# san-soucie/gdrf

Measured on AMD Instinct MI355X. Metric: ELBO steps/sec (+ achieved HBM GB/s on K_nm) at N=1e6,M=512,K=10,V=50, higher is better.
Workload: dtype f32

## Files before the change

gdrf_amd/csrc/api.hip:

```cpp
#include "../../include/gdrf_hip.h"
#include "common.h"
#include "gemm_nt.h"
#include "gemm_tn.h"
#include "gemm_split.h"
#include "gemm_tn_topics.h"
#include "gemm_tn_topics1.h"
#include "kernels_mm.h"
#include "kernels_n.h"
#include "predict.h"
#include "rows_mfma.h"
#include "rows_vstream.h"
#include "hyper_tn.h"
#include "optim.h"

#include <algorithm>
#include <cmath>
#include <cstdio>
#include <cstdlib>
#include <cstring>
#include <string>
#include <type_traits>
#include <vector>

using namespace gdrf;
// ... 950 lines not shown
    if (mask & SL_TRANSFORMS) {
      ScopedTimer tm(c, 2, s);
      dim3 g3((Mp + 255) / 256, Mp, K);
      hipLaunchKernelGGL(build_s_kernel<T>, g3, dim3(256), 0, s, Sunc, M, Mp, P(c->S), P(c->ST));
      hipLaunchKernelGGL(build_phi_kernel<T>, dim3(K), dim3(64), 0, s, phi_unc, K, V, P(c->phi));
      if (c->unwhitened) {
        if ((rc = unwhiten_forward(c, U, s))) return rc;
        U = (const T*)c->Uw;
      }
      hipLaunchKernelGGL(build_upad_kernel<T>, dim3((Mp + 255) / 256, GDRF_TILE), dim3(256), 0, s, U, K, M, Mp, P(c->Upad));
      if (!c->Tst && (rc = mm_nt<T>(c, P(c->S), mm, P(c->S), mm, P(c->Bm), mm, T(1), K, s))) return rc;
      if constexpr (std::is_same<T, float>::value) {
        if (c->split) {
          const SplitLay SL{K};
          HIPCHK(hipMemsetAsync(c->smx, 0, (size_t)SL.nmax() * sizeof(unsigned), s));
          if (c->split == 2) {
            hipLaunchKernelGGL(absmax_batched_kernel, dim3(64, K), dim3(256), 0, s, (const float*)c->Bm, mm, mm, c->smx + SL.mx_b(0));
            hipLaunchKernelGGL(absmax_batched_kernel, dim3(64, K), dim3(256), 0, s, (const float*)c->ST, mm, mm, c->smx + SL.mx_st(0));
          }
          split_scales(c, SPLIT_SC_W | SPLIT_SC_BST, s);
        }
      }
    }
    const int64_t rtiles = (n + GDRF_TILE - 1) / GDRF_TILE;
    if (mask & SL_FORWARD) {
    {
      if ((rc = knm_solve(c, X, n, s))) return rc;
      if ((rc = join_fact(c, s))) return rc;
      ScopedTimer tm(c, 3, s);
      FwdWProb<TS, T> p{{}, {}, (const TS*)Q(c->Knm), n, Mp, (const TS*)Q(c->Linv), P(c->W), P(c->qpart), ldk};
      if (c->split && sizeof(TS) == 8 && sizeof(T) == 4) {
        p.Wh = c->Wh; p.wh_stride = (int64_t)c->ncap * Mp; p.wh_mode = c->split; p.wh_scale = c->ssc + SplitLay{K}.w();
      }
      hipLaunchKernelGGL((gemm_nt_kernel<TS, FwdWProb<TS, T>>), dim3(nt_xcd_row_grid(rtiles, nct<TS>(c))), dim3(256), CS::LDS_BYTES, s, p);
    }
    HIPCHK(hipEventRecord(c->ev_fork, s));
    HIPCHK(hipStreamWaitEvent(c->side, c->ev_fork, 0));
    {
      ScopedTimer tm(c, 4, c->side);
      const size_t ulds = (size_t)K * Mp * sizeof(T);
      if (K <= LOC_KMAX && Mp % (16 * Vec16<T>::N) == 0 && ulds <= 150 * 1024) {
        if (ulds > 48 * 1024) HIPCHK(hipFuncSetAttribute((const void*)loc_rows_kernel<T>, hipFuncAttributeMaxDynamicSharedMemorySize, (int)ulds));
        const int64_t blocks = std::min<int64_t>((n + 31) / 32, 256 * 8);
        hipLaunchKernelGGL(loc_rows_kernel<T>, dim3((unsigned)blocks), dim3(256), ulds, c->side, (const T*)P(c->W), n, Mp, K, (const T*)P(c->Upad), P(c->loc), ldk);
      } else {
        bool wide = false;
        if constexpr (sizeof(T) == 8) {
          if (K > C::CW) {
            LocProb<T, true> p{{}, {}, {}, P(c->W), n, Mp, K, P(c->Upad), P(c->loc), ldk};
            hipLaunchKernelGGL((gemm_nt_kernel<T, LocProb<T, true>>), dim3((unsigned)rtiles), dim3(256), C::LDS_BYTES, c->side, p);
            wide = true;
          }
        }
        if (!wide) {
          LocProb<T> p{{}, {}, {}, P(c->W), n, Mp, K, P(c->Upad), P(c->loc), ldk};
          hipLaunchKernelGGL((gemm_nt_kernel<T, LocProb<T>>), dim3((unsigned)rtiles), dim3(256), C::LDS_BYTES, c->side, p);
        }
      }
    }
    HIPCHK(hipEventRecord(c->ev_loc, c->side));
    if constexpr (std::is_same<T, float>::value && sizeof(TS) == 8) {
      if (hyper_tn_on(c) && !(mask & SL_NO_DK)) {
        const int vpr = Mp / 8, rpp = 256 / vpr;
        const int64_t blocks = std::min<int64_t>((n + rpp - 1) / rpp, 256 * 16);
        if (!c->dKh) {
          void* pw = nullptr;
          hipError_t e = hipMalloc(&pw, (size_t)2 * c->ncap * Mp * 2);
// ... 133 lines not shown
        dim3 gr1((Mp + 255) / 256, Mp, 1);
        hipLaunchKernelGGL(reduce_slabs_kernel<T>, gr1, dim3(256), 0, ss, (const T*)slab_gt, ns, 1, Mp, 0, redT + roff(c, 3)); }
    }
    HIPCHK(hipEventRecord(c->ev_join, c->side));
    bool hyper_done = false;
    if constexpr (std::is_same<T, float>::value && sizeof(TS) == 8) {
      if (hyper_tn_on(c)) {
        hipStream_t ss = c->side;
        ScopedTimer tm(c, 8, ss);
        const int BR = TNCfg<T>::BR;
        const int ns = std::min(tn_nsplit_gt(c, n, BR), c->nsplit_cap);
        const int64_t rps = round_up((n + ns - 1) / ns, BR);
        float* slab_hd = (float*)c->slab + (int64_t)c->nsplit_cap * (K + 1) * mm;
        const SplitLay SL{K};
        if ((rc = tn_split<SplitF16>(c, (const float*)c->Wbar, nullptr, 0, n, rps, 0, slab_hd, 1, ns, c->nt * c->nt, SL.wbar(), 0, ss, c->dKh, SL.dk()))) return rc;
        hipLaunchKernelGGL(slab_linvt_dot_kernel<TS>, dim3((unsigned)M), dim3(256), 0, ss, (const float*)slab_hd, ns, Mp, M, (const TS*)Q(c->LinvT), c->hpart);
        hipLaunchKernelGGL(reduce_dparts_kernel, dim3(1), dim3(1024), 0, ss, c->hpart, (int64_t)M, 1, redd + 5);
        hipLaunchKernelGGL(wbar_w_dot_kernel<T>, dim3(2048), dim3(256), 0, ss, (const T*)P(c->Wbar), (const T*)P(c->W), n, Mp, c->hpart + Mp);
        hipLaunchKernelGGL(reduce_dparts_kernel, dim3(1), dim3(1024), 0, ss, c->hpart + Mp, (int64_t)2048, 1, redd + 4);
        HIPCHK(hipMemsetAsync(redd + 6, 0, sizeof(double), ss));
        LAUNCHCHK("hyper_tn");
        HIPCHK(hipEventRecord(c->ev_join, c->side));
        hyper_done = true;
      }
    }
    if (!hyper_done) {
      ScopedTimer tm(c, 8, s);
      const int64_t nb = nt_xcd_row_grid(rtiles, nct<TS>(c));
      if (3 * nb > c->dpart_len) return fail(-1, "gdrf_step_local", "n_local exceeds the context capacity");
      if (c->per) {
        if (c->learn_z) {
          BwdKnmProb<TS, T, true, true, true> p{{}, {}, P(c->Wbar), n, M, Mp, c->D, c->kind, (const TS*)Q(c->LinvT), (const TS*)Q(c->Knm), X,
                                                (const TS*)Q(c->Zs), c->hyp, c->dpart, c->zpart, c->apart, Xr, (const TS*)Q(c->Zph)};
          hipLaunchKernelGGL((gemm_nt_kernel<TS, BwdKnmProb<TS, T, true, true, true>>), dim3((unsigned)nb), dim3(256), CS::LDS_BYTES, s, p);
          hipLaunchKernelGGL(reduce_parts_kernel<double>, dim3((unsigned)((M * c->D + 255) / 256)), dim3(256), 0, s, (const double*)c->zpart, rtiles,
                             (int64_t)M * c->D, redd + 8);
        } else {
          BwdKnmProb<TS, T, false, true, true> p{{}, {}, P(c->Wbar), n, M, Mp, c->D, c->kind, (const TS*)Q(c->LinvT), (const TS*)Q(c->Knm), X,
                                                 (const TS*)Q(c->Zs), c->hyp, c->dpart, nullptr, c->apart, Xr, (const TS*)Q(c->Zph)};
          if (sizeof(TS) == 8)
            hipLaunchKernelGGL((gemm_nt_kernel_v160<TS, BwdKnmProb<TS, T, false, true, true>>), dim3((unsigned)nb), dim3(256), CS::LDS_BYTES, s, p);
          else hipLaunchKernelGGL((gemm_nt_kernel<TS, BwdKnmProb<TS, T, false, true, true>>), dim3((unsigned)nb), dim3(256), CS::LDS_BYTES, s, p);
        }
        hipLaunchKernelGGL(reduce_dparts_kernel, dim3(1), dim3(1024), 0, s, c->apart, nb, c->D + c->npair, redd + 8 + (int64_t)M * c->D);
      } else if (c->ard) {
        if (c->learn_z) {
          BwdKnmProb<TS, T, true, true> p{{}, {}, P(c->Wbar), n, M, Mp, c->D, c->kind, (const TS*)Q(c->LinvT), (const TS*)Q(c->Knm), X, (const TS*)Q(c->Zs),
                                          c->hyp, c->dpart, c->zpart, c->apart};
          hipLaunchKernelGGL((gemm_nt_kernel<TS, BwdKnmProb<TS, T, true, true>>), dim3((unsigned)nb), dim3(256), CS::LDS_BYTES, s, p);
          hipLaunchKernelGGL(reduce_parts_kernel<double>, dim3((unsigned)((M * c->D + 255) / 256)), dim3(256), 0, s, (const double*)c->zpart, rtiles,
                             (int64_t)M * c->D, redd + 8);
        } else {
          BwdKnmProb<TS, T, false, true> p{{}, {}, P(c->Wbar), n, M, Mp, c->D, c->kind, (const TS*)Q(c->LinvT), (const TS*)Q(c->Knm), X, (const TS*)Q(c->Zs),
                                           c->hyp, c->dpart, nullptr, c->apart};
          if (sizeof(TS) == 8) hipLaunchKernelGGL((gemm_nt_kernel_v160<TS, BwdKnmProb<TS, T, false, true>>), dim3((unsigned)nb), dim3(256), CS::LDS_BYTES, s, p);
          else hipLaunchKernelGGL((gemm_nt_kernel<TS, BwdKnmProb<TS, T, false, true>>), dim3((unsigned)nb), dim3(256), CS::LDS_BYTES, s, p);
        }
        hipLaunchKernelGGL(reduce_dparts_kernel, dim3(1), dim3(1024), 0, s, c->apart, nb, c->D, redd + 8 + (int64_t)M * c->D);
      } else if (c->learn_z) {
        BwdKnmProb<TS, T, true> p{{}, {}, P(c->Wbar), n, M, Mp, c->D, c->kind, (const TS*)Q(c->LinvT), (const TS*)Q(c->Knm), X, (const TS*)Q(c->Zs),
                                  c->hyp, c->dpart, c->zpart};
        hipLaunchKernelGGL((gemm_nt_kernel<TS, BwdKnmProb<TS, T, true>>), dim3((unsigned)nb), dim3(256), CS::LDS_BYTES, s, p);
        hipLaunchKernelGGL(reduce_parts_kernel<double>, dim3((unsigned)((M * c->D + 255) / 256)), dim3(256), 0, s, (const double*)c->zpart, rtiles,
                           (int64_t)M * c->D, redd + 8);
      } else {
        BwdKnmProb<TS, T> p{{}, {}, P(c->Wbar), n, M, Mp, c->D, c->kind, (const TS*)Q(c->LinvT), (const TS*)Q(c->Knm), X, (const TS*)Q(c->Zs), c->hyp,
                            c->dpart, nullptr};
        if (sizeof(TS) == 8) hipLaunchKernelGGL((gemm_nt_kernel_v160<TS, BwdKnmProb<TS, T>>), dim3((unsigned)nb), dim3(256), CS::LDS_BYTES, s, p);
        else hipLaunchKernelGGL((gemm_nt_kernel<TS, BwdKnmProb<TS, T>>), dim3((unsigned)nb), dim3(256), CS::LDS_BYTES, s, p);
      }
      hipLaunchKernelGGL(reduce_dparts_kernel, dim3(1), dim3(1024), 0, s, c->dpart, nb, 3, redd + 4);
    }
    LAUNCHCHK("backward");
    {
      const int BR = TNCfg<T>::BR;
      const int ns = std::min(tn_nsplit(c, n, BR, c->split ? 2 : 3), c->nsplit_cap);
      const int64_t rps = round_up((n + ns - 1) / ns, BR);
      TNArgs<T> a{P(c->W), Mp, P(c->W), Mp, P(c->vbar), ldk, n, rps, Mp, 1, P(c->slab), K, ns};
      int red_ns = ns, red_qd = GDRF_TILE / 2;
      { ScopedTimer tm(c, 9, s);
        if (c->split == 2) {
          if constexpr (std::is_same<T, float>::value) {
            const SplitLay SL{K};
            const int nst = std::min(tn_topics_nsplit(c, n), c->nsplit_cap);
            const int64_t rpst = round_up((n + nst - 1) / nst, 32);
            const int ntl = tnt_ntiles(Mp), kgroups = (K + TNT_KT - 1) / TNT_KT;
            TNTopicsArgs ta{(const _Float16*)c->Wh, (int64_t)c->ncap * Mp, Mp, (const float*)c->W, Mp, (const float*)c->vbar, ldk, n, rpst, Mp,
                            (float*)c->slab, K, nst, ntl, (const float*)c->ssc, SL.w(), SL.v(0)};
            if (10 * K >= 6 * kgroups * TNT_KT) {
              int ns1 = c->nsplit_cap < 64 ? c->nsplit_cap : 64;
              while (ns1 > 8 && (n + ns1 - 1) / ns1 < 8 * TN1_CH) ns1 -= 8;
              if (ns1 >= 8) ns1 &= ~7;
              const int64_t rps1 = round_up((n + ns1 - 1) / ns1, TN1_CH);
              const int64_t lds64 = round_up(c->ncap, 64);
              hipLaunchKernelGGL(tn1_scale_rows_kernel, dim3(256, K), dim3(256), 0, s, (const float*)c->vbar, ldk, n, (float*)c->vbs, lds64,
                                 (const float*)c->ssc, SL.v(0));
              TNTopicsArgs t1{(const _Float16*)c->Wh, (int64_t)c->ncap * Mp, Mp, (const float*)c->W, Mp, (const float*)c->vbs, lds64, n, rps1, Mp,
                              (float*)c->slab, K, ns1, ntl, (const float*)c->ssc, SL.w(), SL.v(0)};
              const int nth = tn2_ntiles_half(Mp);
              TNTopicsArgs t0 = t1, t4 = t1;
              t0.ntiles = ntl - nth; t4.ntiles = nth;
              HIPCHK(hipFuncSetAttribute((const void*)tn_topics_w2_kernel<0>, hipFuncAttributeMaxDynamicSharedMemorySize, tn2_lds_bytes()));
// ... 587 lines not shown
```

gdrf_amd/csrc/common.h:

```cpp
#pragma once
#include <hip/hip_runtime.h>
#include <stdint.h>

#define GDRF_WAVE 64
#define GDRF_TILE 128
#define GDRF_KBYTES 128
#define GDRF_FWDW_WGS 2
#define GDRF_FWDW_DEPTH 2
#define GDRF_MPAD 32
#define GDRF_DMAX 4

namespace gdrf {

template <typename T> struct Vec16;
template <> struct Vec16<float>  { using type = float  __attribute__((ext_vector_type(4))); static constexpr int N = 4; };
template <> struct Vec16<double> { using type = double __attribute__((ext_vector_type(2))); static constexpr int N = 2; };

template <typename T> struct Mfma;
template <> struct Mfma<float> {
  using acc_t = float __attribute__((ext_vector_type(4)));
  static __device__ __forceinline__ acc_t mma(float a, float b, acc_t c) {
    return __builtin_amdgcn_mfma_f32_16x16x4f32(a, b, c, 0, 0, 0);
  }
  static __device__ __forceinline__ int crow(int lane, int r) { return ((lane >> 4) << 2) + r; }
};
template <> struct Mfma<double> {
  using acc_t = double __attribute__((ext_vector_type(4)));
  static __device__ __forceinline__ acc_t mma(double a, double b, acc_t c) {
    return __builtin_amdgcn_mfma_f64_16x16x4f64(a, b, c, 0, 0, 0);
  }
  static __device__ __forceinline__ int crow(int lane, int r) { return (lane >> 4) + (r << 2); }
};

__device__ __forceinline__ void gdrf_raw_barrier() {
  asm volatile("" ::: "memory");
  __builtin_amdgcn_s_barrier();
  asm volatile("" ::: "memory");
}

template <typename T> __device__ __forceinline__ T wave_sum(T v) {
#pragma unroll
  for (int o = 32; o > 0; o >>= 1) v += __shfl_xor(v, o, 64);
  return v;
}
template <typename T> __device__ __forceinline__ T group16_sum(T v) {
// ... 81 lines not shown
```

gdrf_amd/csrc/gemm_nt.h:

```cpp
#pragma once
#include "common.h"

namespace gdrf {

template <typename T> struct NTCfg {
  static constexpr int BK = GDRF_KBYTES / (int)sizeof(T);
  static constexpr int VE = 16 / (int)sizeof(T);
  static constexpr int LDK = BK + VE;
  static constexpr int KG = BK / 4;
  static constexpr int VPR = BK / VE;
  static constexpr int VPT = GDRF_TILE * VPR / 256;
  static constexpr int CW = sizeof(T) == 4 ? 128 : 64;
  static constexpr int NB = CW / 32;
  static constexpr int VPTB = CW * VPR / 256;
  static constexpr int LDS_BYTES = (GDRF_TILE + CW) * LDK * (int)sizeof(T);
};

template <typename T> __device__ __forceinline__ int nt_stage_row(int i) { return (int)(threadIdx.x / NTCfg<T>::VPR) + (256 / NTCfg<T>::VPR) * i; }
template <typename T> __device__ __forceinline__ int nt_stage_k() { return (int)(threadIdx.x % NTCfg<T>::VPR) * NTCfg<T>::VE; }

template <class P, class = void> struct NTTri { static constexpr int value = 0; };
template <class P> struct NTTri<P, decltype((void)P::TRI)> { static constexpr int value = P::TRI; };

template <class P, class = void> struct NTMinWgs { static constexpr int value = 2; };
template <class P> struct NTMinWgs<P, decltype((void)P::MIN_WGS)> { static constexpr int value = P::MIN_WGS; };

template <typename T, class P> __device__ __forceinline__ void gemm_nt_body(P& p);

template <typename T, class P>
__global__ __launch_bounds__(256, NTMinWgs<P>::value) void gemm_nt_kernel(P p) { gemm_nt_body<T, P>(p); }

template <typename T, class P>
__global__ __launch_bounds__(256, 3) __attribute__((amdgpu_num_vgpr(80))) void gemm_nt_kernel_v160(P p) { gemm_nt_body<T, P>(p); }

template <typename T, class P>
__device__ __forceinline__ void gemm_nt_body(P& p) {
  using C = NTCfg<T>;
  using V = typename Vec16<T>::type;
  using MM = Mfma<T>;
  using acc_t = typename MM::acc_t;
  extern __shared__ __attribute__((aligned(16))) char smem[];
  T* As = reinterpret_cast<T*>(smem);
  T* Bs = As + GDRF_TILE * C::LDK;
  char* extra = smem + C::LDS_BYTES;

  const int tid = threadIdx.x, lane = tid & 63, wave = tid >> 6;
  const int wr = wave >> 1, wc = wave & 1, lr = lane & 15, lg = lane >> 4;
  const int wc_u = __builtin_amdgcn_readfirstlane(wc);
  const int nct = p.col_tiles();
  const bool loopc = p.loop_cols();
  int64_t rtile; int ct_first;
  p.map_block(blockIdx.x, nct, loopc, rtile, ct_first);
  const int ct_last = loopc ? nct : ct_first + 1;
  const int64_t m0 = rtile * GDRF_TILE;
  const int bz = p.batch_index(blockIdx.x, blockIdx.y);
  const int R = p.a_reuse();

  typename P::ACtx actx;
  p.prepA(actx, m0, bz, extra);
  typename P::ECtx ectx;
  p.prepE(ectx, m0, bz);
  const T* scaleS = reinterpret_cast<const T*>(extra);

  const int srow_k = nt_stage_k<T>();
  for (int ct = ct_first; ct < ct_last; ++ct) {
    const int n0 = ct * C::CW;
    acc_t acc[4][C::NB];
#pragma unroll
    for (int a = 0; a < 4; ++a)
#pragma unroll
      for (int b = 0; b < C::NB; ++b) acc[a][b] = acc_t{0, 0, 0, 0};
    int kb, ke;
    p.krange(m0, n0, bz, kb, ke);
    const int nchunks = (ke > kb) ? ((ke - kb) / C::BK) * R : 0;
    const int nk = (ke > kb) ? (ke - kb) / C::BK : 0;
    auto chunk_pos = [&](int c, int& kA, int& rep) {
      if (P::A_PER_REP) { rep = c / nk; kA = kb + (c - rep * nk) * C::BK; }
      else { const int q = c / R; rep = c - q * R; kA = kb + q * C::BK; }
    };
    typename P::AVec ra0[C::VPT], ra1[C::VPT];
    V rb0[C::VPTB], rb1[C::VPTB];
    auto gload = [&](typename P::AVec (&ra)[C::VPT], V (&rb)[C::VPTB], int c) {
      int kA, rep;
      chunk_pos(c, kA, rep);
      if (rep == 0 || P::A_PER_REP) {
#pragma unroll
        for (int i = 0; i < C::VPT; ++i) ra[i] = p.loadA(actx, i, kA + srow_k, rep, bz);
      }
#pragma unroll
      for (int i = 0; i < C::VPTB; ++i) rb[i] = p.loadB(n0, i, kA + srow_k, rep, bz);
    };
    auto compute = [&](int rep, int kA = 0) {
      T sc[4];
      bool need[C::NB];
#pragma unroll
      for (int b = 0; b < C::NB; ++b) {
        const int c0 = n0 + wc_u * (C::CW / 2) + b * 16;
        need[b] = NTTri<P>::value == 1 ? (kA <= c0 + 15) : (NTTri<P>::value == 2 ? (kA + C::BK - 1 >= c0) : true);
      }
      if (P::SCALE_A) {
#pragma unroll
        for (int t4 = 0; t4 < 4; ++t4) sc[t4] = rep >= 0 ? scaleS[rep * GDRF_TILE + wr * 64 + t4 * 16 + lr] : T(1);
      }
      const T* pa = &As[(wr * 64 + lr) * C::LDK + lg * C::KG];
      const T* pb = &Bs[(wc * (C::CW / 2) + lr) * C::LDK + lg * C::KG];
#pragma unroll
      for (int v = 0; v < C::KG / C::VE; ++v) {
        V fa[4], fb[C::NB];
#pragma unroll
        for (int t4 = 0; t4 < 4; ++t4) {
          fa[t4] = *reinterpret_cast<const V*>(pa + t4 * 16 * C::LDK + v * C::VE);
          if (P::SCALE_A) {
#pragma unroll
            for (int e = 0; e < C::VE; ++e) fa[t4][e] *= sc[t4];
          }
        }
#pragma unroll
        for (int t4 = 0; t4 < C::NB; ++t4) fb[t4] = *reinterpret_cast<const V*>(pb + t4 * 16 * C::LDK + v * C::VE);
#pragma unroll
        for (int e = 0; e < C::VE; ++e)
#pragma unroll
          for (int a = 0; a < 4; ++a)
#pragma unroll
            for (int b = 0; b < C::NB; ++b) {
              if (NTTri<P>::value == 0 || need[b]) acc[a][b] = MM::mma(fa[a][e], fb[b][e], acc[a][b]);
            }
      }
    };
    auto body = [&](typename P::AVec (&ra)[C::VPT], V (&rb)[C::VPTB], int c) {
      int kA, rep;
      chunk_pos(c, kA, rep);
      __syncthreads();
      if (rep == 0 || P::A_PER_REP) {
#pragma unroll
        for (int i = 0; i < C::VPT; ++i) *reinterpret_cast<V*>(&As[nt_stage_row<T>(i) * C::LDK + srow_k]) = p.a_to_lds(ra[i], actx, i, kA + srow_k);
      }
#pragma unroll
      for (int i = 0; i < C::VPTB; ++i) *reinterpret_cast<V*>(&Bs[nt_stage_row<T>(i) * C::LDK + srow_k]) = rb[i];
      __syncthreads();
      if (c + P::DEPTH < nchunks) gload(ra, rb, c + P::DEPTH);
      compute(rep, kA);
    };
    if (P::DEPTH == 1) {
      if (nchunks > 0) gload(ra0, rb0, 0);
      for (int c = 0; c < nchunks; ++c) body(ra0, rb0, c);
    } else {
      if (nchunks > 0) gload(ra0, rb0, 0);
      if (nchunks > 1) gload(ra1, rb1, 1);
      for (int c = 0; c < nchunks; c += 2) {
        body(ra0, rb0, c);
        if (c + 1 < nchunks) body(ra1, rb1, c + 1);
      }
    }
    for (int x = 0; x < p.extra_chunks(); ++x) {
      __syncthreads();
      p.fill_extra(As, Bs, x, m0, n0);
      __syncthreads();
      compute(-1);
    }
    p.tile_done(acc, m0, n0, bz, ectx, wr, wc, lane);
  }
  p.finish(m0, bz, ectx, smem, wr, wc, lane);
}

template <typename T> __device__ __forceinline__ int nt_acc_row(int wr, int a, int lane, int r) {
  return wr * 64 + a * 16 + Mfma<T>::crow(lane, r);
}
template <typename T> __device__ __forceinline__ int nt_acc_col(int wc, int b, int lane) {
  return wc * (NTCfg<T>::CW / 2) + b * 16 + (lane & 15);
}

template <typename T> struct NTPlainA {
  using AVec = typename Vec16<T>::type;
  template <class... X> __device__ __forceinline__ AVec a_to_lds(const AVec& v, X&&...) const { return v; }
};
struct NTNoExtra {
  __device__ __forceinline__ int extra_chunks() const { return 0; }
  template <typename T> __device__ __forceinline__ void fill_extra(T*, T*, int, int64_t, int) const {}
};

struct NTDefaultMap {
  __device__ __forceinline__ int batch_index(unsigned, unsigned by) const { return (int)by; }
  __device__ __forceinline__ void map_block(unsigned bid, int nct, bool loopc, int64_t& rtile, int& ct) const {
    if (loopc) { rtile = bid; ct = 0; } else { rtile = bid / nct; ct = (int)(bid % nct); }
  }
};
struct NTXcdMap {
  __device__ __forceinline__ int batch_index(unsigned, unsigned by) const { return (int)by; }
  __device__ __forceinline__ void map_block(unsigned bid, int nct, bool loopc, int64_t& rtile, int& ct) const {
    if (loopc) { rtile = bid; ct = 0; return; }
    if (nct > 8 || (8 % nct) != 0 || (gridDim.x % 8u) != 0) { rtile = bid / nct; ct = (int)(bid % nct); return; }
    const unsigned xcd = bid & 7u, idx = bid >> 3, per = 8u / (unsigned)nct;
    ct = (int)(xcd % (unsigned)nct);
    rtile = (int64_t)idx * per + xcd / (unsigned)nct;
  }
};

inline unsigned nt_xcd_row_grid(int64_t rtiles, int nct) { return (unsigned)(8 * nct * ((rtiles + 7) / 8)); }
struct NTXcdRowMap {
  __device__ __forceinline__ int batch_index(unsigned, unsigned by) const { return (int)by; }
  __device__ __forceinline__ void map_block(unsigned bid, int nct, bool loopc, int64_t& rtile, int& ct) const {
    if (loopc) { rtile = bid; ct = 0; return; }
    const unsigned xcd = bid & 7u, idx = bid >> 3;
    rtile = (int64_t)(idx / (unsigned)nct) * 8 + xcd;
    ct = (int)(idx % (unsigned)nct);
    if ((nct & 3) == 0 && ((idx >> 2) & 1u)) ct = (ct & ~3) + 3 - (ct & 3);
  }
};

struct NTXcdRowBatchMap {
  int nbatch;
  __device__ __forceinline__ int batch_index(unsigned bid, unsigned) const { return (int)((bid >> 3) % (unsigned)nbatch); }
// ... 51 lines not shown
```

gdrf_amd/csrc/gemm_split.h:

```cpp
#pragma once
#include "common.h"
#include "gemm_nt.h"
#include "kernels_mm.h"

namespace gdrf {

typedef __bf16 bf16x8 __attribute__((ext_vector_type(8)));
typedef __bf16 bf16x4 __attribute__((ext_vector_type(4)));
typedef _Float16 f16x8 __attribute__((ext_vector_type(8)));
typedef _Float16 f16x4 __attribute__((ext_vector_type(4)));
typedef float f32x4 __attribute__((ext_vector_type(4)));
typedef uint32_t u32x4 __attribute__((ext_vector_type(4)));

struct SplitBf16 {
  using E = __bf16; using V8 = bf16x8; using V4 = bf16x4;
  static constexpr int NP = 3, NPROD = 6, ID = 1;
  static __device__ __forceinline__ constexpr int pa(int t) { constexpr int v[6] = {0, 1, 2, 0, 1, 0}; return v[t]; }
  static __device__ __forceinline__ constexpr int pb(int t) { constexpr int v[6] = {2, 1, 0, 1, 0, 0}; return v[t]; }
  static __device__ __forceinline__ f32x4 mma(V8 a, V8 b, f32x4 c) { return __builtin_amdgcn_mfma_f32_16x16x32_bf16(a, b, c, 0, 0, 0); }
  static __device__ __forceinline__ void split(float x, E (&p)[NP]) {
    p[0] = (__bf16)x;
    const float r1 = x - (float)p[0];
    p[1] = (__bf16)r1;
    p[2] = (__bf16)(r1 - (float)p[1]);
// ... 45 lines not shown
  if ((what & SPLIT_SC_WBAR) && t == 0) put(L.wbar(), f16 ? split_pow2_scale(__uint_as_float(mx[L.mx_wbar()]), 15) : 1.0f);
  for (int k = t; k < K; k += blockDim.x) {
    if (what & SPLIT_SC_BST) {
      put(L.b(k), f16 ? split_pow2_scale(__uint_as_float(mx[L.mx_b(k)]), 15) : 1.0f);
      put(L.st(k), f16 ? split_pow2_scale(__uint_as_float(mx[L.mx_st(k)]), 15) : 1.0f);
    }
    if (what & SPLIT_SC_V) put(L.v(k), f16 ? split_pow2_scale(__uint_as_float(mx[L.mx_v(k)]) * sqrtf((float)h->var), 13) : 1.0f);
  }
}
__global__ __launch_bounds__(256) void absmax_batched_kernel(const float* __restrict__ x, int64_t n, int64_t ld, unsigned* __restrict__ mx) {
  const int b = blockIdx.y;
  float m = 0;
  const f32x4* p = reinterpret_cast<const f32x4*>(x + (int64_t)b * ld);
  for (int64_t i = (int64_t)blockIdx.x * blockDim.x + threadIdx.x; i < (n >> 2); i += (int64_t)gridDim.x * blockDim.x) {
    const f32x4 v = p[i];
    m = fmaxf(fmaxf(m, fmaxf(fabsf(v[0]), fabsf(v[1]))), fmaxf(fabsf(v[2]), fabsf(v[3])));
  }
  if (blockIdx.x == 0 && threadIdx.x < (n & 3)) m = fmaxf(m, fabsf(x[(int64_t)b * ld + (n & ~(int64_t)3) + threadIdx.x]));
#pragma unroll
  for (int o = 32; o > 0; o >>= 1) m = fmaxf(m, __shfl_xor(m, o, 64));
  if ((threadIdx.x & 63) == 0 && m > 0) atomicMax(mx + b, __float_as_uint(m));
}

template <class SP> struct SplitCfg {
  static constexpr int BK = 32;
  static constexpr int LDH = BK;
  static constexpr int PIECE = GDRF_TILE * LDH;
  static constexpr int IMG = SP::NP * PIECE;
  static constexpr int LDS_BYTES = 2 * IMG * 2;
};
__device__ __forceinline__ int split_swz(int row) { return (row & 8) ? 3 : 0; }
__device__ __forceinline__ int split_off(int row, int k) { return row * 32 + (((k >> 3) ^ split_swz(row)) << 3) + (k & 7); }

__device__ __forceinline__ void glds16_asm(const void* gsrc, unsigned lds_dst) {
  asm volatile("s_mov_b32 m0, %1\n\ts_nop 0\n\tglobal_load_lds_dwordx4 %0, off" : : "v"(gsrc), "s"(lds_dst) : "memory");
}
__device__ __forceinline__ void glds16_asm_s(const void* sbase, unsigned voff, unsigned lds_dst) {
  asm volatile("s_mov_b32 m0, %2\n\ts_nop 0\n\tglobal_load_lds_dwordx4 %0, %1" : : "v"(voff), "s"(sbase), "s"(lds_dst) : "memory");
}
__device__ __forceinline__ unsigned lds_addr(const void* p) {
  return (unsigned)(uintptr_t)(__attribute__((address_space(3))) const void*)p;
}


template <class SP>
__global__ void split_kernel(const float* __restrict__ in, int64_t n, typename SP::E* __restrict__ out, int64_t stride, const float* __restrict__ scale) {
  const int64_t i = ((int64_t)blockIdx.x * blockDim.x + threadIdx.x) * 4;
  if (i >= n) return;
  const float s = scale[0];
  const f32x4 x = *reinterpret_cast<const f32x4*>(in + i);
  typename SP::V4 pv[SP::NP];
#pragma unroll
  for (int e = 0; e < 4; ++e) {
    typename SP::E p[SP::NP];
    SP::split(x[e] * s, p);
#pragma unroll
    for (int q = 0; q < SP::NP; ++q) pv[q][e] = p[q];
  }
#pragma unroll
  for (int q = 0; q < SP::NP; ++q) *reinterpret_cast<typename SP::V4*>(out + q * stride + i) = pv[q];
}

template <class SP>
__global__ void split_blocked_kernel(const float* __restrict__ in, int64_t n, int R, int C, typename SP::E* __restrict__ out, int64_t stride,
                                     const float* __restrict__ scale) {
  const int64_t i = ((int64_t)blockIdx.x * blockDim.x + threadIdx.x) * 4;
  if (i >= n) return;
  const int64_t rc = (int64_t)R * C, b = i / rc, rem = i - b * rc;
  const float s = scale[2 * b];
  const f32x4 x = *reinterpret_cast<const f32x4*>(in + i);
  typename SP::V4 pv[SP::NP];
#pragma unroll
  for (int e = 0; e < 4; ++e) {
    typename SP::E p[SP::NP];
    SP::split(x[e] * s, p);
// ... 1157 lines not shown
```

gdrf_amd/csrc/kernels_n.h:

```cpp
#pragma once
#include "common.h"
#include "gemm_nt.h"
#include "kernels_mm.h"
#include "gemm_split.h"


namespace gdrf {

template <typename T> __device__ __forceinline__ typename Vec16<T>::type vzero() {
  typename Vec16<T>::type z;
#pragma unroll
  for (int e = 0; e < Vec16<T>::N; ++e) z[e] = 0;
  return z;
}

template <typename T> __device__ __forceinline__ T cov_fast(int kind, T r2, T var, T alpha);

__constant__ double exp2_coef[13] = {1.0, 0.6931471805599453, 0.2402265069591007, 0.055504108664821576, 0.009618129107628477, 0.0013333558146428441, 0.00015403530393381606, 1.5252733804059838e-05, 1.3215486790144305e-06, 1.0178086009239696e-07, 7.054911620801121e-09, 4.44553827187081e-10, 2.5678435993488196e-11};
__device__ __forceinline__ double exp2_poly(double t) {
  t = fmax(t, -1100.0);
  const double k = __builtin_rint(t), r = t - k;
  double p = exp2_coef[12];
#pragma unroll
  for (int i = 11; i >= 0; --i) p = fma(p, r, exp2_coef[i]);
// ... 565 lines not shown
      const int kk = e / GDRF_TILE, row = e - kk * GDRF_TILE, k = x * BK + kk;
      As[row * LDK + kk] = (k < K && m0 + row < nrows) ? locbar[(int64_t)k * ldk + m0 + row] : T(0);
    }
    for (int e = threadIdx.x; e < CW * BK; e += 256) {
      const int kk = e / CW, col = e - kk * CW, k = x * BK + kk;
      Bs[col * LDK + kk] = (k < K && n0 + col < M) ? U[(int64_t)k * M + n0 + col] : T(0);
    }
  }
  template <class Acc, int NB_>
  __device__ __forceinline__ void tile_done(Acc (&acc)[4][NB_], int64_t m0, int n0, int, ECtx&, int wr, int wc, int lane) const {
#pragma unroll
    for (int a = 0; a < 4; ++a)
#pragma unroll
      for (int r = 0; r < 4; ++r) {
        const int64_t m = m0 + nt_acc_row<T>(wr, a, lane, r);
        if (m >= nrows) continue;
        const T as2 = T(2) * asum[m];
#pragma unroll
        for (int b = 0; b < NTCfg<T>::NB; ++b) {
          const int n = n0 + nt_acc_col<T>(wc, b, lane);
          if (n >= Mp) continue;
          T v = acc[a][b][r] - as2 * W[m * Mp + n];
          Wbar[m * Mp + n] = v;
        }
      }
  }
  __device__ __forceinline__ void finish(int64_t, int, ECtx&, char*, int, int, int) const {}
};

template <typename T, typename TN, bool LZ = false, bool ARD = false, bool PER = false> struct BwdKnmProb : NTXcdRowMap, NTNoExtra {
  using V = typename Vec16<T>::type;
  static constexpr int MIN_WGS = (sizeof(T) == 8 && !LZ) ? 3 : 2;
  static constexpr int TRI = 2;
  static constexpr bool SCALE_A = false;
  static constexpr bool A_PER_REP = false;
  static constexpr int DEPTH = 1;
  const TN* Wbar; int64_t nrows; int M, Mp, D, kind;
  const T* LinvT;
  const T* Knm;
  const TN* X; const T* Z; const Hyper* h;
  double* part;
  double* zpart;
  double* apart = nullptr;
  const TN* Xr = nullptr; const T* Zph = nullptr;
  struct ACtx { const TN* p[NTCfg<T>::VPT]; };
  struct ECtxIso { T s1, s2, s3; T zs[LZ ? NTCfg<T>::NB : 1][LZ ? GDRF_DMAX : 1]; int n0; };
  struct ECtxArd : ECtxIso { T sd[GDRF_DMAX]; };
  struct ECtxPer : ECtxArd { T pd[GDRF_DMAX / 2]; };
  using ECtx = std::conditional_t<PER, ECtxPer, std::conditional_t<ARD, ECtxArd, ECtxIso>>;
  __device__ __forceinline__ int col_tiles() const { return (Mp + NTCfg<T>::CW - 1) / NTCfg<T>::CW; }
  __device__ __forceinline__ bool loop_cols() const { return false; }
  __device__ __forceinline__ int a_reuse() const { return 1; }
  __device__ __forceinline__ void krange(int64_t, int n0, int, int& kb, int& ke) const { kb = n0; ke = Mp; }
  __device__ __forceinline__ void prepA(ACtx& c, int64_t m0, int, char*) const {
#pragma unroll
    for (int i = 0; i < NTCfg<T>::VPT; ++i) {
      const int64_t r = m0 + nt_stage_row<T>(i);
      c.p[i] = (r < nrows) ? Wbar + r * Mp : nullptr;
    }
  }
  __device__ __forceinline__ void prepE(ECtx& e, int64_t, int) const {
    e.s1 = 0; e.s2 = 0; e.s3 = 0; e.n0 = 0;
    if constexpr (ARD) {
#pragma unroll
      for (int d = 0; d < GDRF_DMAX; ++d) e.sd[d] = 0;
    }
    if constexpr (PER) {
#pragma unroll
      for (int d = 0; d < GDRF_DMAX / 2; ++d) e.pd[d] = 0;
    }
    if constexpr (LZ) {
#pragma unroll
      for (int b = 0; b < NTCfg<T>::NB; ++b)
#pragma unroll
        for (int d = 0; d < GDRF_DMAX; ++d) e.zs[b][d] = 0;
    }
  }
  using AVec = TN __attribute__((ext_vector_type(Vec16<T>::N)));
  __device__ __forceinline__ AVec loadA(const ACtx& c, int i, int k, int, int) const {
    AVec t;
#pragma unroll
    for (int e = 0; e < Vec16<T>::N; ++e) t[e] = 0;
    if (c.p[i]) t = *reinterpret_cast<const AVec*>(c.p[i] + k);
    return t;
  }
  template <class... X> __device__ __forceinline__ V a_to_lds(const AVec& t, X&&...) const {
    V v;
#pragma unroll
    for (int e = 0; e < Vec16<T>::N; ++e) v[e] = (T)t[e];
    return v;
  }
  __device__ __forceinline__ V loadB(int n0, int i, int k, int, int) const {
    const int c = n0 + nt_stage_row<T>(i);
    return (c < Mp) ? *reinterpret_cast<const V*>(LinvT + (int64_t)c * Mp + k) : vzero<T>();
  }
  typedef T KT2 __attribute__((ext_vector_type(2)));
  template <int KD, int DD, int NR>
  __device__ __forceinline__ void strip_math(const KT2 (&kv)[NR], const T* __restrict__ trow, int tstride, const TN (&x)[NR][DD],
                                             const T (&zc)[2][DD], const bool (&rok)[NR], const bool (&cok)[2],
                                             T ils2, T al, ECtx& e, const T (&xsc)[DD], const T (&px)[NR], const T (&pz)[2]) const {
#pragma unroll
    for (int i = 0; i < NR; ++i) {
      const KT2 kb = *reinterpret_cast<const KT2*>(trow + 4 * i * tstride);
#pragma unroll
      for (int j = 0; j < 2; ++j) {
        const T kbar = (rok[i] && cok[j]) ? kb[j] : T(0);
        const T kvv = kv[i][j];
        T r2 = 0;
#pragma unroll
        for (int d = 0; d < DD; ++d) { const T t = (d < D ? (ARD ? (T)x[i][d] * xsc[d] : (T)x[i][d]) : T(0)) - zc[j][d]; r2 += t * t; }
        r2 *= ils2;
        e.s1 += kbar * kvv;
        if constexpr (ARD) {
          const T w = T(-2) * kbar * dcov_dr2_from_k<T>(KD, kvv, r2, al);
#pragma unroll
          for (int d = 0; d < DD; ++d) { const T t = (d < D ? (T)x[i][d] * xsc[d] : T(0)) - zc[j][d]; e.sd[d] += w * t * t; }
          if constexpr (PER) e.pd[0] += w * (px[i] - pz[j]) * ((T)x[i][1] * zc[j][0] - (T)x[i][0] * zc[j][1]);
        } else {
          e.s2 += kbar * dcov_dlogls_from_k<T>(KD, kvv, r2, al);
        }
        if constexpr (KD == 4) e.s3 += kbar * dcov_dlogalpha_from_k<T>(KD, kvv, r2, al);
        if constexpr (LZ) {
          const T w = kbar * dcov_dr2_from_k<T>(KD, kvv, r2, al);
#pragma unroll
          for (int d = 0; d < DD; ++d) e.zs[j][d] += w * (zc[j][d] - (d < D ? (ARD ? (T)x[i][d] * xsc[d] : (T)x[i][d]) : T(0)));
        }
      }
    }
// ... 1076 lines not shown
```

Measured before the change: 25.04.

## Stage backward Knm GEMM operands via LDS-DMA loads with swizzled double buffer

Adds a new GEMM body for the backward Knm kernel that copies A (Wbar) and B (LinvT) tiles straight from global memory into LDS using global_load_lds_dwordx4. It uses a two-stage ring with XOR swizzling and skips triangular column blocks at the MFMA level. The aim is to remove the register round trip and the explicit LDS stores in the staging path. It only applies when the accumulation type is f64 (DMA = sizeof(T)==8), so with f32 state it runs only if the shared-precision type TS is double. Launch sites now size dynamic LDS per problem type, and the DMA helpers move into common.h.

```diff
diff --git a/gdrf_amd/csrc/api.hip b/gdrf_amd/csrc/api.hip
--- a/gdrf_amd/csrc/api.hip
+++ b/gdrf_amd/csrc/api.hip
@@ -1006,7 +1006,7 @@
       if (c->split && sizeof(TS) == 8 && sizeof(T) == 4) {
         p.Wh = c->Wh; p.wh_stride = (int64_t)c->ncap * Mp; p.wh_mode = c->split; p.wh_scale = c->ssc + SplitLay{K}.w();
       }
-      hipLaunchKernelGGL((gemm_nt_kernel<TS, FwdWProb<TS, T>>), dim3(nt_xcd_row_grid(rtiles, nct<TS>(c))), dim3(256), CS::LDS_BYTES, s, p);
+      hipLaunchKernelGGL((gemm_nt_kernel<TS, FwdWProb<TS, T>>), dim3(nt_xcd_row_grid(rtiles, nct<TS>(c))), dim3(256), (nt_lds_bytes<TS, FwdWProb<TS, T>>()), s, p);
     }
     HIPCHK(hipEventRecord(c->ev_fork, s));
     HIPCHK(hipStreamWaitEvent(c->side, c->ev_fork, 0));
@@ -1206,42 +1206,42 @@
         if (c->learn_z) {
           BwdKnmProb<TS, T, true, true, true> p{{}, {}, P(c->Wbar), n, M, Mp, c->D, c->kind, (const TS*)Q(c->LinvT), (const TS*)Q(c->Knm), X,
                                                 (const TS*)Q(c->Zs), c->hyp, c->dpart, c->zpart, c->apart, Xr, (const TS*)Q(c->Zph)};
-          hipLaunchKernelGGL((gemm_nt_kernel<TS, BwdKnmProb<TS, T, true, true, true>>), dim3((unsigned)nb), dim3(256), CS::LDS_BYTES, s, p);
+          hipLaunchKernelGGL((gemm_nt_kernel<TS, BwdKnmProb<TS, T, true, true, true>>), dim3((unsigned)nb), dim3(256), (nt_lds_bytes<TS, BwdKnmProb<TS, T, true, true, true>>()), s, p);
           hipLaunchKernelGGL(reduce_parts_kernel<double>, dim3((unsigned)((M * c->D + 255) / 256)), dim3(256), 0, s, (const double*)c->zpart, rtiles,
                              (int64_t)M * c->D, redd + 8);
         } else {
           BwdKnmProb<TS, T, false, true, true> p{{}, {}, P(c->Wbar), n, M, Mp, c->D, c->kind, (const TS*)Q(c->LinvT), (const TS*)Q(c->Knm), X,
                                                  (const TS*)Q(c->Zs), c->hyp, c->dpart, nullptr, c->apart, Xr, (const TS*)Q(c->Zph)};
           if (sizeof(TS) == 8)
-            hipLaunchKernelGGL((gemm_nt_kernel_v160<TS, BwdKnmProb<TS, T, false, true, true>>), dim3((unsigned)nb), dim3(256), CS::LDS_BYTES, s, p);
-          else hipLaunchKernelGGL((gemm_nt_kernel<TS, BwdKnmProb<TS, T, false, true, true>>), dim3((unsigned)nb), dim3(256), CS::LDS_BYTES, s, p);
+            hipLaunchKernelGGL((gemm_nt_kernel_v160<TS, BwdKnmProb<TS, T, false, true, true>>), dim3((unsigned)nb), dim3(256), (nt_lds_bytes<TS, BwdKnmProb<TS, T, false, true, true>>()), s, p);
+          else hipLaunchKernelGGL((gemm_nt_kernel<TS, BwdKnmProb<TS, T, false, true, true>>), dim3((unsigned)nb), dim3(256), (nt_lds_bytes<TS, BwdKnmProb<TS, T, false, true, true>>()), s, p);
         }
         hipLaunchKernelGGL(reduce_dparts_kernel, dim3(1), dim3(1024), 0, s, c->apart, nb, c->D + c->npair, redd + 8 + (int64_t)M * c->D);
       } else if (c->ard) {
         if (c->learn_z) {
           BwdKnmProb<TS, T, true, true> p{{}, {}, P(c->Wbar), n, M, Mp, c->D, c->kind, (const TS*)Q(c->LinvT), (const TS*)Q(c->Knm), X, (const TS*)Q(c->Zs),
                                           c->hyp, c->dpart, c->zpart, c->apart};
-          hipLaunchKernelGGL((gemm_nt_kernel<TS, BwdKnmProb<TS, T, true, true>>), dim3((unsigned)nb), dim3(256), CS::LDS_BYTES, s, p);
+          hipLaunchKernelGGL((gemm_nt_kernel<TS, BwdKnmProb<TS, T, true, true>>), dim3((unsigned)nb), dim3(256), (nt_lds_bytes<TS, BwdKnmProb<TS, T, true, true>>()), s, p);
           hipLaunchKernelGGL(reduce_parts_kernel<double>, dim3((unsigned)((M * c->D + 255) / 256)), dim3(256), 0, s, (const double*)c->zpart, rtiles,
                              (int64_t)M * c->D, redd + 8);
         } else {
           BwdKnmProb<TS, T, false, true> p{{}, {}, P(c->Wbar), n, M, Mp, c->D, c->kind, (const TS*)Q(c->LinvT), (const TS*)Q(c->Knm), X, (const TS*)Q(c->Zs),
                                            c->hyp, c->dpart, nullptr, c->apart};
-          if (sizeof(TS) == 8) hipLaunchKernelGGL((gemm_nt_kernel_v160<TS, BwdKnmProb<TS, T, false, true>>), dim3((unsigned)nb), dim3(256), CS::LDS_BYTES, s, p);
-          else hipLaunchKernelGGL((gemm_nt_kernel<TS, BwdKnmProb<TS, T, false, true>>), dim3((unsigned)nb), dim3(256), CS::LDS_BYTES, s, p);
+          if (sizeof(TS) == 8) hipLaunchKernelGGL((gemm_nt_kernel_v160<TS, BwdKnmProb<TS, T, false, true>>), dim3((unsigned)nb), dim3(256), (nt_lds_bytes<TS, BwdKnmProb<TS, T, false, true>>()), s, p);
+          else hipLaunchKernelGGL((gemm_nt_kernel<TS, BwdKnmProb<TS, T, false, true>>), dim3((unsigned)nb), dim3(256), (nt_lds_bytes<TS, BwdKnmProb<TS, T, false, true>>()), s, p);
         }
         hipLaunchKernelGGL(reduce_dparts_kernel, dim3(1), dim3(1024), 0, s, c->apart, nb, c->D, redd + 8 + (int64_t)M * c->D);
       } else if (c->learn_z) {
         BwdKnmProb<TS, T, true> p{{}, {}, P(c->Wbar), n, M, Mp, c->D, c->kind, (const TS*)Q(c->LinvT), (const TS*)Q(c->Knm), X, (const TS*)Q(c->Zs),
                                   c->hyp, c->dpart, c->zpart};
-        hipLaunchKernelGGL((gemm_nt_kernel<TS, BwdKnmProb<TS, T, true>>), dim3((unsigned)nb), dim3(256), CS::LDS_BYTES, s, p);
+        hipLaunchKernelGGL((gemm_nt_kernel<TS, BwdKnmProb<TS, T, true>>), dim3((unsigned)nb), dim3(256), (nt_lds_bytes<TS, BwdKnmProb<TS, T, true>>()), s, p);
         hipLaunchKernelGGL(reduce_parts_kernel<double>, dim3((unsigned)((M * c->D + 255) / 256)), dim3(256), 0, s, (const double*)c->zpart, rtiles,
                            (int64_t)M * c->D, redd + 8);
       } else {
         BwdKnmProb<TS, T> p{{}, {}, P(c->Wbar), n, M, Mp, c->D, c->kind, (const TS*)Q(c->LinvT), (const TS*)Q(c->Knm), X, (const TS*)Q(c->Zs), c->hyp,
                             c->dpart, nullptr};
-        if (sizeof(TS) == 8) hipLaunchKernelGGL((gemm_nt_kernel_v160<TS, BwdKnmProb<TS, T>>), dim3((unsigned)nb), dim3(256), CS::LDS_BYTES, s, p);
-        else hipLaunchKernelGGL((gemm_nt_kernel<TS, BwdKnmProb<TS, T>>), dim3((unsigned)nb), dim3(256), CS::LDS_BYTES, s, p);
+        if (sizeof(TS) == 8) hipLaunchKernelGGL((gemm_nt_kernel_v160<TS, BwdKnmProb<TS, T>>), dim3((unsigned)nb), dim3(256), (nt_lds_bytes<TS, BwdKnmProb<TS, T>>()), s, p);
+        else hipLaunchKernelGGL((gemm_nt_kernel<TS, BwdKnmProb<TS, T>>), dim3((unsigned)nb), dim3(256), (nt_lds_bytes<TS, BwdKnmProb<TS, T>>()), s, p);
       }
       hipLaunchKernelGGL(reduce_dparts_kernel, dim3(1), dim3(1024), 0, s, c->dpart, nb, 3, redd + 4);
     }
diff --git a/gdrf_amd/csrc/common.h b/gdrf_amd/csrc/common.h
--- a/gdrf_amd/csrc/common.h
+++ b/gdrf_amd/csrc/common.h
@@ -11,6 +11,16 @@
 #define GDRF_DMAX 4
 
 namespace gdrf {
+
+__device__ __forceinline__ void glds16_asm(const void* gsrc, unsigned lds_dst) {
+  asm volatile("s_mov_b32 m0, %1\n\ts_nop 0\n\tglobal_load_lds_dwordx4 %0, off" : : "v"(gsrc), "s"(lds_dst) : "memory");
+}
+__device__ __forceinline__ void glds16_asm_s(const void* sbase, unsigned voff, unsigned lds_dst) {
+  asm volatile("s_mov_b32 m0, %2\n\ts_nop 0\n\tglobal_load_lds_dwordx4 %0, %1" : : "v"(voff), "s"(sbase), "s"(lds_dst) : "memory");
+}
+__device__ __forceinline__ unsigned lds_addr(const void* p) {
+  return (unsigned)(uintptr_t)(__attribute__((address_space(3))) const void*)p;
+}
 
 template <typename T> struct Vec16;
 template <> struct Vec16<float>  { using type = float  __attribute__((ext_vector_type(4))); static constexpr int N = 4; };
diff --git a/gdrf_amd/csrc/gemm_nt.h b/gdrf_amd/csrc/gemm_nt.h
--- a/gdrf_amd/csrc/gemm_nt.h
+++ b/gdrf_amd/csrc/gemm_nt.h
@@ -1,4 +1,5 @@
 #pragma once
+#include <type_traits>
 #include "common.h"
 
 namespace gdrf {
@@ -21,10 +22,37 @@
 
 template <class P, class = void> struct NTTri { static constexpr int value = 0; };
 template <class P> struct NTTri<P, decltype((void)P::TRI)> { static constexpr int value = P::TRI; };
+template <typename T, class P> __device__ __forceinline__ bool nt_tri_need(int kA, int c0) {
+  return NTTri<P>::value == 1 ? (kA <= c0 + 15) : (NTTri<P>::value == 2 ? (kA + NTCfg<T>::BK - 1 >= c0) : true);
+}
 
 template <class P, class = void> struct NTMinWgs { static constexpr int value = 2; };
 template <class P> struct NTMinWgs<P, decltype((void)P::MIN_WGS)> { static constexpr int value = P::MIN_WGS; };
 
+template <class P, class = void> struct NTDma { static constexpr bool value = false; };
+template <class P> struct NTDma<P, decltype((void)P::DMA)> { static constexpr bool value = P::DMA; };
+
+template <typename T, typename TA> struct NTDmaCfg {
+  static constexpr int AROW = NTCfg<T>::BK * (int)sizeof(TA);
+  static constexpr int AQ = AROW / 16;
+  static constexpr int BROW = NTCfg<T>::BK * (int)sizeof(T);
+  static constexpr int A_BYTES = GDRF_TILE * AROW;
+  static constexpr int B_BYTES = NTCfg<T>::CW * BROW;
+  static constexpr int STAGE = A_BYTES + B_BYTES;
+  static constexpr int RING = 2;
+  static constexpr int LDS_BYTES = RING * STAGE;
+  static constexpr int AREQ = A_BYTES / 4096;
+  static constexpr int BREQ = B_BYTES / 4096;
+  static_assert(BROW == 128 && A_BYTES % 4096 == 0 && B_BYTES % 4096 == 0, "LDS-DMA staging: 16 k per chunk, whole requests per wave");
+};
+template <int QPR> __device__ __forceinline__ int nt_swz(int r) { return QPR == 8 ? ((r >> 1) & 5) : ((r >> 2) & 2); }
+
+template <typename T, class P> constexpr int nt_lds_bytes() {
+  if constexpr (NTDma<P>::value) return NTDmaCfg<T, typename P::AStage>::LDS_BYTES;
+  else return NTCfg<T>::LDS_BYTES;
+}
+
+template <typename T, class P> __device__ __forceinline__ void gemm_nt_dma_body(P& p);
 template <typename T, class P> __device__ __forceinline__ void gemm_nt_body(P& p);
 
 template <typename T, class P>
@@ -35,6 +63,10 @@
 
 template <typename T, class P>
 __device__ __forceinline__ void gemm_nt_body(P& p) {
+  if constexpr (NTDma<P>::value) {
+    gemm_nt_dma_body<T, P>(p);
+    return;
+  }
   using C = NTCfg<T>;
   using V = typename Vec16<T>::type;
   using MM = Mfma<T>;
@@ -90,14 +122,11 @@
 #pragma unroll
       for (int i = 0; i < C::VPTB; ++i) rb[i] = p.loadB(n0, i, kA + srow_k, rep, bz);
     };
-    auto compute = [&](int rep, int kA = 0) {
+    auto compute = [&](int rep, int kA, bool tri) {
       T sc[4];
       bool need[C::NB];
 #pragma unroll
-      for (int b = 0; b < C::NB; ++b) {
-        const int c0 = n0 + wc_u * (C::CW / 2) + b * 16;
-        need[b] = NTTri<P>::value == 1 ? (kA <= c0 + 15) : (NTTri<P>::value == 2 ? (kA + C::BK - 1 >= c0) : true);
-      }
+      for (int b = 0; b < C::NB; ++b) need[b] = !tri || nt_tri_need<T, P>(kA, n0 + wc_u * (C::CW / 2) + b * 16);
       if (P::SCALE_A) {
 #pragma unroll
         for (int t4 = 0; t4 < 4; ++t4) sc[t4] = rep >= 0 ? scaleS[rep * GDRF_TILE + wr * 64 + t4 * 16 + lr] : T(1);
@@ -139,7 +168,7 @@
       for (int i = 0; i < C::VPTB; ++i) *reinterpret_cast<V*>(&Bs[nt_stage_row<T>(i) * C::LDK + srow_k]) = rb[i];
       __syncthreads();
       if (c + P::DEPTH < nchunks) gload(ra, rb, c + P::DEPTH);
-      compute(rep, kA);
+      compute(rep, kA, true);
     };
     if (P::DEPTH == 1) {
       if (nchunks > 0) gload(ra0, rb0, 0);
@@ -156,7 +185,7 @@
       __syncthreads();
       p.fill_extra(As, Bs, x, m0, n0);
       __syncthreads();
-      compute(-1);
+      compute(-1, 0, false);
     }
     p.tile_done(acc, m0, n0, bz, ectx, wr, wc, lane);
   }
@@ -178,6 +207,128 @@
   __device__ __forceinline__ int extra_chunks() const { return 0; }
   template <typename T> __device__ __forceinline__ void fill_extra(T*, T*, int, int64_t, int) const {}
 };
+
+template <typename T, class P>
+__device__ __forceinline__ void gemm_nt_dma_body(P& p) {
+  using C = NTCfg<T>;
+  using TA = typename P::AStage;
+  using D = NTDmaCfg<T, TA>;
+  using V = typename Vec16<T>::type;
+  using MM = Mfma<T>;
+  using acc_t = typename MM::acc_t;
+  static_assert(C::NB == 2, "LDS-DMA staging: the f64 column tile (two MFMA columns per wave)");
+  static_assert(!P::SCALE_A && !P::A_PER_REP && std::is_base_of<NTNoExtra, P>::value, "LDS-DMA staging: plain problems only");
+  extern __shared__ __attribute__((aligned(16))) char smem[];
+  const int tid = threadIdx.x, lane = tid & 63, wave = tid >> 6;
+  const int wr = wave >> 1, wc = wave & 1, lr = lane & 15, lg = lane >> 4;
+  const int wc_u = __builtin_amdgcn_readfirstlane(wc), wave_u = __builtin_amdgcn_readfirstlane(wave);
+  const int nct = p.col_tiles();
+  int64_t rtile; int ct;
+  p.map_block(blockIdx.x, nct, false, rtile, ct);
+  const int64_t m0 = rtile * GDRF_TILE;
+  const int n0 = ct * C::CW;
+  const int bz = p.batch_index(blockIdx.x, blockIdx.y);
+  const int Mp = p.Mp;
+  const int64_t nrows = p.nrows;
+  typename P::ECtx ectx;
+  p.prepE(ectx, m0, bz);
+
+  const int64_t arow0 = m0 < nrows ? m0 : nrows - 1;
+  const TA* Ag = p.a_src() + arow0 * Mp;
+  const T* Bg = p.b_src() + (int64_t)n0 * Mp;
+  unsigned aoff[D::AREQ], boff[D::BREQ];
+#pragma unroll
+  for (int i = 0; i < D::AREQ; ++i) {
+    const int row = (wave * D::AREQ + i) * (1024 / D::AROW) + lane / D::AQ;
+    const int64_t gr = m0 + row < nrows ? m0 + row : nrows - 1;
+    aoff[i] = (unsigned)((gr - arow0) * Mp * (int64_t)sizeof(TA)) + (unsigned)(((lane % D::AQ) ^ nt_swz<D::AQ>(row & 15)) * 16);
+  }
+#pragma unroll
+  for (int i = 0; i < D::BREQ; ++i) {
+    const int row = (wave * D::BREQ + i) * 8 + (lane >> 3);
+    const int c = n0 + row < Mp ? n0 + row : Mp - 1;
+    boff[i] = (unsigned)((int64_t)(c - n0) * Mp * (int64_t)sizeof(T)) + (unsigned)(((lane & 7) ^ nt_swz<8>(row & 15)) * 16);
+  }
+  const unsigned lds0 = lds_addr(smem);
+
+  acc_t acc[4][C::NB];
+#pragma unroll
+  for (int a = 0; a < 4; ++a)
+#pragma unroll
+    for (int b = 0; b < C::NB; ++b) acc[a][b] = acc_t{0, 0, 0, 0};
+  int kb, ke;
+  p.krange(m0, n0, bz, kb, ke);
+  const int nch = ke > kb ? (ke - kb) / C::BK : 0;
+  auto issue = [&](int c) {
+    const int kA = kb + c * C::BK;
+    const unsigned st = lds0 + (unsigned)((c % D::RING) * D::STAGE);
+#pragma unroll
+    for (int i = 0; i < D::AREQ; ++i) glds16_asm_s(Ag + kA, aoff[i], st + (unsigned)((wave_u * D::AREQ + i) * 1024));
+#pragma unroll
+    for (int i = 0; i < D::BREQ; ++i) glds16_asm_s(Bg + kA, boff[i], st + (unsigned)(D::A_BYTES + (wave_u * D::BREQ + i) * 1024));
+  };
+  const int sw = nt_swz<8>(lr), swa = nt_swz<D::AQ>(lr);
+  auto compute = [&](int c) {
+    const int kA = kb + c * C::BK;
+    const char* st = smem + (c % D::RING) * D::STAGE;
+    const char* pa = st + (wr * 64 + lr) * D::AROW;
+    const char* pb = st + D::A_BYTES + (wc * (C::CW / 2) + lr) * D::BROW;
+    V fa[2][4], fb[2][C::NB];
+#pragma unroll
+    for (int t4 = 0; t4 < 4; ++t4) {
+      if constexpr (D::AQ == 8) {
+#pragma unroll
+        for (int v = 0; v < 2; ++v) fa[v][t4] = *reinterpret_cast<const V*>(pa + t4 * 16 * D::AROW + (((2 * lg + v) ^ swa) << 4));
+      } else {
+        typedef TA ta4 __attribute__((ext_vector_type(4)));
+        const ta4 f = *reinterpret_cast<const ta4*>(pa + t4 * 16 * D::AROW + ((lg ^ swa) << 4));
+#pragma unroll
+        for (int v = 0; v < 2; ++v) { fa[v][t4][0] = (T)f[2 * v]; fa[v][t4][1] = (T)f[2 * v + 1]; }
+      }
+    }
+#pragma unroll
+    for (int t4 = 0; t4 < C::NB; ++t4)
+#pragma unroll
+      for (int v = 0; v < 2; ++v) fb[v][t4] = *reinterpret_cast<const V*>(pb + t4 * 16 * D::BROW + (((2 * lg + v) ^ sw) << 4));
+    auto mma_cols = [&](auto lo_, auto hi_) {
+      constexpr int lo = decltype(lo_)::value, hi = decltype(hi_)::value;
+#pragma unroll
+      for (int v = 0; v < 2; ++v)
+#pragma unroll
+        for (int e = 0; e < C::VE; ++e)
+#pragma unroll
+          for (int a = 0; a < 4; ++a)
+#pragma unroll
+            for (int b = lo; b < hi; ++b) acc[a][b] = MM::mma(fa[v][a][e], fb[v][b][e], acc[a][b]);
+    };
+    using I0 = std::integral_constant<int, 0>;
+    using I1 = std::integral_constant<int, 1>;
+    using I2 = std::integral_constant<int, 2>;
+    if constexpr (NTTri<P>::value == 0) {
+      mma_cols(I0{}, I2{});
+    } else {
+      const int c0 = n0 + wc_u * (C::CW / 2);
+      const bool n0_ = nt_tri_need<T, P>(kA, c0), n1_ = nt_tri_need<T, P>(kA, c0 + 16);
+      if (n0_ && n1_) mma_cols(I0{}, I2{});
+      else if (n0_) mma_cols(I0{}, I1{});
+      else if (n1_) mma_cols(I1{}, I2{});
+    }
+  };
+  if (nch > 0) issue(0);
+  for (int c = 0; c < nch; ++c) {
+    asm volatile("s_waitcnt vmcnt(0) lgkmcnt(0)\n\ts_barrier" ::: "memory");
+    if (c + 1 < nch) issue(c + 1);
+    compute(c);
+  }
+#pragma unroll
+  for (int b = 0; b < C::NB; ++b)
+    if (n0 + nt_acc_col<T>(wc, b, lane) >= Mp) {
+#pragma unroll
+      for (int a = 0; a < 4; ++a) acc[a][b] = acc_t{0, 0, 0, 0};
+    }
+  p.tile_done(acc, m0, n0, bz, ectx, wr, wc, lane);
+  p.finish(m0, bz, ectx, smem, wr, wc, lane);
+}
 
 struct NTDefaultMap {
   __device__ __forceinline__ int batch_index(unsigned, unsigned by) const { return (int)by; }
diff --git a/gdrf_amd/csrc/gemm_split.h b/gdrf_amd/csrc/gemm_split.h
--- a/gdrf_amd/csrc/gemm_split.h
+++ b/gdrf_amd/csrc/gemm_split.h
@@ -101,15 +101,6 @@
 __device__ __forceinline__ int split_swz(int row) { return (row & 8) ? 3 : 0; }
 __device__ __forceinline__ int split_off(int row, int k) { return row * 32 + (((k >> 3) ^ split_swz(row)) << 3) + (k & 7); }
 
-__device__ __forceinline__ void glds16_asm(const void* gsrc, unsigned lds_dst) {
-  asm volatile("s_mov_b32 m0, %1\n\ts_nop 0\n\tglobal_load_lds_dwordx4 %0, off" : : "v"(gsrc), "s"(lds_dst) : "memory");
-}
-__device__ __forceinline__ void glds16_asm_s(const void* sbase, unsigned voff, unsigned lds_dst) {
-  asm volatile("s_mov_b32 m0, %2\n\ts_nop 0\n\tglobal_load_lds_dwordx4 %0, %1" : : "v"(voff), "s"(sbase), "s"(lds_dst) : "memory");
-}
-__device__ __forceinline__ unsigned lds_addr(const void* p) {
-  return (unsigned)(uintptr_t)(__attribute__((address_space(3))) const void*)p;
-}
 
 
 template <class SP>
diff --git a/gdrf_amd/csrc/kernels_n.h b/gdrf_amd/csrc/kernels_n.h
--- a/gdrf_amd/csrc/kernels_n.h
+++ b/gdrf_amd/csrc/kernels_n.h
@@ -621,6 +621,8 @@
   using V = typename Vec16<T>::type;
   static constexpr int MIN_WGS = (sizeof(T) == 8 && !LZ) ? 3 : 2;
   static constexpr int TRI = 2;
+  static constexpr bool DMA = sizeof(T) == 8;
+  using AStage = TN;
   static constexpr bool SCALE_A = false;
   static constexpr bool A_PER_REP = false;
   static constexpr int DEPTH = 1;
@@ -683,6 +685,8 @@
     const int c = n0 + nt_stage_row<T>(i);
     return (c < Mp) ? *reinterpret_cast<const V*>(LinvT + (int64_t)c * Mp + k) : vzero<T>();
   }
+  __device__ __forceinline__ const TN* a_src() const { return Wbar; }
+  __device__ __forceinline__ const T* b_src() const { return LinvT; }
   typedef T KT2 __attribute__((ext_vector_type(2)));
   template <int KD, int DD, int NR>
   __device__ __forceinline__ void strip_math(const KT2 (&kv)[NR], const T* __restrict__ trow, int tstride, const TN (&x)[NR][DD],
```

Result: faster. 25.34, median of 6 (+1.2%).
